# Sir-Teo/MuZero-Go

Measured on AMD Instinct MI355X. Metric: MCTS simulations/sec (whole node) + self-play moves/sec, 9x9 Go, 200 sims/move, higher is better.
Workload: dtype fp32

## Files before the change

include/mzgo.h:

```cpp
#ifndef MZGO_H
#define MZGO_H

#include <stdint.h>

#ifdef __cplusplus
extern "C" {
#endif

enum {
  MZGO_OK = 0,
  MZGO_EINVAL = -1,
  MZGO_EHIP = -2,
  MZGO_ENOWEIGHTS = -3,
  MZGO_EASSERT = -4
};

typedef struct mzgo_config {
  int board_size;
  int latent_dim;
  int num_games;
  int num_simulations;
  int max_moves;
  int compat;
  int temperature_moves;
// ... 45 lines not shown
int mzgo_board_reset(mzgo_engine* eng, void* stream);
int mzgo_board_step(mzgo_engine* eng, const int32_t* actions, int32_t* status, double* winner,
                    void* stream);
int mzgo_board_planes(mzgo_engine* eng, double* planes, void* stream);
int mzgo_board_set(mzgo_engine* eng, int g, const int8_t* stones_host, const uint8_t* invd_host,
                   const int32_t* meta_host, void* stream);

int mzgo_selfplay_reset(mzgo_engine* eng, int epoch, void* stream);
int mzgo_selfplay_move(mzgo_engine* eng, void* stream);
int mzgo_selfplay_moves(mzgo_engine* eng, int moves, void* stream);

int mzgo_arena_move(mzgo_engine* eng, mzgo_engine* opponent, void* stream);
int mzgo_arena_moves(mzgo_engine* eng, mzgo_engine* opponent, int moves, void* stream);
int mzgo_selfplay_counters(mzgo_engine* eng, uint64_t* counters_host, void* stream);
int mzgo_search_stats(mzgo_engine* eng, uint64_t* stats_host, void* stream);

int mzgo_selfplay_set_timing(mzgo_engine* eng, int on);
int mzgo_selfplay_launch_times(mzgo_engine* eng, float* boards_ms, float* queue_ms, int cap, int* n_host);
int mzgo_stream_wait_started(mzgo_engine* eng, uint64_t target, void* stream);
int mzgo_tower_timing(mzgo_engine* eng, int enable, double* tower_ms_host, int64_t* towers_host);

int mzgo_dyn_conv_backward_workspace(int B, int C, int64_t* bytes_host);
int mzgo_dyn_conv_backward(const float* grad_out, const float* out, const float* latent, const int64_t* action,
                           const float* emb, const float* weight, int B, int C, int N, float* grad_latent,
                           float* grad_weight, float* grad_bias, void* workspace, int64_t workspace_bytes,
                           void* stream);
int mzgo_conv3x3_relu_forward(const float* x, const int64_t* action, const float* emb, const float* weight,
                              const float* bias, int B, int Cin, int Cout, int N, float* out, void* stream);
int mzgo_conv3x3_backward_workspace(int B, int Cin, int Cout, int64_t* bytes_host);
int mzgo_conv3x3_backward(const float* grad_out, const float* out, const float* x, const int64_t* action,
// ... 67 lines not shown
```

muzero-go_amd/csrc/mzgo_capi.hip:

```cpp
#include <hip/hip_runtime.h>

#include <algorithm>
#include <cmath>
#include <cstdarg>
#include <cstdio>
#include <cstring>
#include <map>
#include <string>
#include <vector>

#include "../../include/mzgo.h"
#include "mzgo_dispatch.hpp"
#include "mzgo_replay.hpp"
#include "mzgo_tower_host.hpp"

namespace mzgo {
extern const KernelSet kernels_n5_c96, kernels_n6_c96, kernels_n9_c96, kernels_n19_c96, kernels_n6_c128,
    kernels_n6_c64;

size_t conv_bwd_workspace_bytes(int B, int Cin, int Cout);
hipError_t conv_forward(const float* x, const int64_t* action, const float* emb, const float* w, const float* bias,
                        int B, int Cin, int Cout, int N, float* y, hipStream_t s);
hipError_t conv_backward(const float* g, const float* out, const float* x, const int64_t* action, const float* emb,
                         const float* w, int B, int Cin, int Cout, int N, float* gx, float* gw, float* gb,
// ... 169 lines not shown
  float* d_w = nullptr;
  size_t d_w_bytes = 0;
  NetParams np{};
  EngineArrays E{};
  int* d_err = nullptr;
  unsigned* rq_head = nullptr;
  float* d_scr = nullptr;
  size_t scr_floats = 0;
  std::vector<void*> allocs;
  bool timing = false;
  std::vector<hipEvent_t> tev;
  int tn = 0;
  int64_t bytes = 0;
  int epoch = 0;
  int value_cache = 0;
  const double* noise = nullptr;
  double* noise_out = nullptr;
  TowerHost* tower = nullptr;

  template <class T>
  int alloc(T** p, size_t n) {
    void* v = nullptr;
    hipError_t e = hipMalloc(&v, n * sizeof(T) + 256);
    if (e != hipSuccess) return fail(MZGO_EHIP, "hipMalloc(%zu): %s", n * sizeof(T), hipGetErrorString(e));
    allocs.push_back(v);
    bytes += (int64_t)(n * sizeof(T));
    *p = reinterpret_cast<T*>(v);
    return MZGO_OK;
  }
  ~mzgo_engine() {
// ... 96 lines not shown

  SearchParams search_params() const {
    SearchParams sp;
    sp.c_puct = cfg.c_puct; sp.discount = cfg.discount;
    sp.dirichlet_alpha = cfg.dirichlet_alpha; sp.dirichlet_epsilon = cfg.dirichlet_epsilon;
    sp.pass_epsilon = cfg.pass_epsilon; sp.num_simulations = S; sp.compat = cfg.compat;
    sp.variant = cfg.search_variant;
    sp.factored = cfg.direct_dynamics ? 0 : 1;
    sp.seed = cfg.seed;
    sp.helpers = 0;
    sp.net = 0;
    sp.tail = 0;
    const char* lz = getenv("MZGO_LAZY_ROWS");
    sp.lazy_rows = lz && atoi(lz) == 0 ? 0 : 1;
    sp.value_cache = value_cache;
    return sp;
  }
};

void mzgo::replay_engine_view(const mzgo_engine* e, ReplayEngineView* v) {
  const EngineArrays& E = e->E;
  *v = ReplayEngineView{e->N, e->G, e->M, e->C, e->tower ? 1 : 0, e->cfg.game_base, e->epoch,
                        E.stones, E.invd, E.meta, E.rec_stones, E.rec_invd, E.rec_flags, E.rec_action,
                        E.rec_value, E.rec_policy, E.rec_reward, E.final_reward};
}

extern "C" {

const char* mzgo_last_error(void) { return g_err.c_str(); }

// ... 119 lines not shown
    }
  }
  if (C != 0) {
    chk(e->alloc(&E.prior, TSL * n1 * A));
    chk(e->alloc(&E.child, TSL * n1 * A));
    chk(e->alloc(&E.visits, TSL * n1));
    chk(e->alloc(&E.wsum, TSL * n1));
    chk(e->alloc(&E.root_prior, TSL * A));
    chk(e->alloc(&E.path, TSL * (n1 + 1)));
    chk(e->alloc(&E.nodes, TSL));
    chk(e->alloc(&E.nact, TSL * n1));
    const char* vc = getenv("MZGO_VALUE_CACHE");
    e->value_cache = !TW && !cfg->direct_dynamics && ks->value_cache_cap > 0 && e->S + 2 <= ks->value_cache_cap &&
                     !(vc && atoi(vc) == 0);
    if (e->value_cache) chk(e->alloc(&E.cval, TSL * n1 * A));
    chk(e->alloc(&E.jobs, TSL * job_bytes(A)));
    chk(e->alloc(&E.mpq, 2 * (size_t)G + 1));
    chk(e->alloc(&E.rec_stones, G * M * CELLS));
    chk(e->alloc(&E.rec_invd, G * M * CELLS));
    chk(e->alloc(&E.rec_flags, G * M));
    chk(e->alloc(&E.rec_action, G * M));
    chk(e->alloc(&E.rec_value, G * M));
    chk(e->alloc(&E.rec_policy, G * M * A));
    chk(e->alloc(&E.rec_reward, G * M));
  }
  chk(e->alloc(&E.stones, G * CELLS));
  chk(e->alloc(&E.invd, G * CELLS));
  chk(e->alloc(&E.meta, G * 4));
  chk(e->alloc(&E.game_len, G));
  chk(e->alloc(&E.final_reward, G));
// ... 499 lines not shown
    return fail(MZGO_EHIP, "mzgo_stream_wait_started: %llu gate(s) gave up before the target count", c[8]);
  }
  return MZGO_OK;
}

int mzgo_search_stats(mzgo_engine* e, uint64_t* out, void* stream) {
  if (!e || !out) return fail(MZGO_EINVAL, "bad argument");
  hipStream_t s = (hipStream_t)stream;
  unsigned long long c[3] = {};
  HIPCHK(hipMemcpyAsync(c, e->E.counters + 9, sizeof c, hipMemcpyDeviceToHost, s));
  HIPCHK(hipStreamSynchronize(s));
  out[0] = c[0]; out[1] = c[1]; out[2] = c[2];
  return MZGO_OK;
}

int mzgo_records_export(mzgo_engine* e, int g, int32_t* length, int32_t* status, int8_t* stones,
                        uint8_t* invd, uint8_t* flags, int32_t* action, double* value, double* policy,
                        double* reward, double* final_reward, void* stream) {
  if (!e || e->C == 0 || g < 0 || g >= e->G) return fail(MZGO_EINVAL, "bad argument");
  hipStream_t s = (hipStream_t)stream;
  int meta[4], st = 0;
  HIPCHK(hipMemcpyAsync(meta, e->E.meta + (size_t)g * 4, 16, hipMemcpyDeviceToHost, s));
  HIPCHK(hipMemcpyAsync(&st, e->E.status + g, 4, hipMemcpyDeviceToHost, s));
  HIPCHK(hipStreamSynchronize(s));
  if (int rc = check_chain(e, s)) return rc;
  const int L = meta[3];
  if (length) *length = L;
  if (status) *status = st;
  const size_t M = e->M, CELLS = e->CELLS, A = e->A, base = (size_t)g * M;
  if (L > 0) {
// ... 64 lines not shown
```

muzero-go_amd/csrc/mzgo_kernels.hpp:

```cpp
#pragma once
#include "mzgo_jobs.hpp"
#include "mzgo_replay.hpp"

namespace mzgo {

template <class G>
constexpr bool rep_needs_scratch() {
  if constexpr (G::WINO) return Wino<G>::NSTRIP > 1;
  else return false;
}

struct NoRepJobs {
  __device__ bool operator()(int) const { return false; }
};

template <class G, class PlaneFn, class Jobs = NoRepJobs>
__device__ __forceinline__ void representation(Smem<G>& sm, const NetParams& np, PlaneFn planes, float* lat,
                                      int lat_stride, float* scr, unsigned long long* ts = nullptr,
                                      Jobs jobs = Jobs{}) {
  float* mid = rep_needs_scratch<G>() ? scr : lat;
  for (int i = tid_local(); i < 6 * G::CELLS; i += G::THREADS) {
    const int c = i / G::CELLS, j = i - c * G::CELLS;
    sm.u.in[c * G::CPAD + j] = planes(c, j);
  }
// ... 814 lines not shown
  int* nact = E.nact + (size_t)g * ((size_t)E.S + 1);
  const int S = sp.num_simulations;
  const bool factored = sp.factored != 0;
  constexpr bool BATCH = decltype(sm.u.f)::BATCH;
  Acc T(TV, sm.t);
  tree_reset_root<G>(T);
  if (tid_local() == 0) {
    sm.t.newest = -1; sm.t.newp_node = -1; sm.t.ycache = -1; sm.t.rowc_node = -1; sm.t.lognode = -1;
  }
  __syncthreads();

  int nodes = 1, convs = 0;
  constexpr bool VCACHE = Acc::LDS && BATCH && decltype(sm.u.f)::CACHE;
  const bool vcache = VCACHE && factored && sp.value_cache != 0 && E.cval != nullptr && !shared_jobs<G>(sp);
  int nbcomp = 0, nbcache = 0, ncut = 0;
  auto cache_cut = [&](int leaf, int m, int B) {
    double* cv = E.cval + ((size_t)g * ((size_t)E.S + 1) + (size_t)leaf) * G::A;
    for (int i = m + tid_local() - 64; tid_local() >= 64 && i < B; i += G::THREADS - 64)
      cv[sm.u.f.acts[i]] = sm.u.f.bv[i];
    if (tid_local() == 0) sm.t.cvm[leaf >> 5] |= 1u << (leaf & 31);
    __syncthreads();
  };
  int rows = 0;
  const bool eager_rows = !(Acc::LDS || shared_jobs<G>(sp) || (decltype(sm.u.f)::GLOBAL_Y && sp.lazy_rows));
  Stamp st(E.stamps);
  int sim = 0;
  if (factored) {
    sim = root_batch<G, Acc>(sm, np, sp, E, g, TV, T, pool, scratch, nact, key, &st);
    if (eager_rows) rows += sim;
    nodes += sim;
// ... 3 lines not shown
  bool pending = false;
  int node0 = 0, depth0 = 0;
  while (sim < S) {
    if (!pending) {
      if (wave_id() == 0) {
        const int a = select_leaf<G>(sm.t, T, sp, key, sim, &st, node0, depth0);
        if (lane_id_local() == 0) sm.t.action = a;
        st.wave_add(92, 1);
        st.wave_add(95, (unsigned long long)sm.t.depth);
      }
      __syncthreads();
    }
    pending = false;
    node0 = 0;
    depth0 = 0;
    while (sm.t.action == kNeedLogits) {
      const int xn = sm.t.leaf, xd = sm.t.depth;
      st.lap(0);
      if (y_lds_target<G>(sm) != nullptr && sm.t.ycache == sm.t.lpar)
        policy_sums_wg<G>(sm.t.logits, sm.u.f.yc, np.etab + (size_t)sm.t.lact * 9 * G::C, sm.u.f.hw);
      else
        policy_sums_wg<G>(sm.t.logits, pool + (size_t)sm.t.lpar * node_floats,
                          np.etab + (size_t)sm.t.lact * 9 * G::C, np.head_w);
      if (tid_local() == 0) sm.t.lognode = xn;
      ++rows;
      __syncthreads();
      st.lap(32);
      if (tid_local() == 0) st.wave_add(34, 1);
      if (wave_id() == 0) {
        const int a = select_leaf<G>(sm.t, T, sp, key, sim, &st, xn, xd);
        if (lane_id_local() == 0) sm.t.action = a;
      }
      __syncthreads();
      st.lap(33);
    }
    st.lap(0);
    const int a = sm.t.action, leaf = sm.t.leaf, depth = sm.t.depth;
    if (a < 0) {
      if (wave_id() == 0 && a == -1) backup<G>(T, depth, -1, 0.0);
      __syncthreads();
      ++sim;
      continue;
    }
    const float* heads;
    const int nid = nodes;
    if (factored) {
      float* yleaf = pool + (size_t)leaf * node_floats;
      int yc = sm.t.ycache;
      bool prepicked = false;
      static_assert(!decltype(sm.u.f)::CACHE || 3 * G::C <= G::THREADS, "one head weight per thread");
      float hwpre = 0.f;
      bool hwready = false;
      if (!sm.t.yready) {
        const bool sj = shared_jobs<G>(sp);
        if (leaf != 0 && !sj && !G::WINO) {
          const int par = T.path(depth - 1);
          materialize<G>(scratch, pool + (size_t)par * node_floats, np.etab + (size_t)nact[leaf] * 9 * G::C,
                         sm.ulds());
        }
        st.lap(81);
        if (sj) {
          const int nun0 = sm.t.nunexp, B0 = BATCH ? (nun0 < S - sim ? nun0 : S - sim) : 1;
          prepicked = BATCH && B0 >= 2;
          conv_shared<G>(sm, np, E, g, leaf, sp.net, &st, leaf != 0 ? T.path(depth - 1) : -1,
                         leaf != 0 ? nact[leaf] : 0, [&](unsigned cb) {
                           if (prepicked && wave_id() == 0) {
                             uint64_t um0[G::AP];
#pragma unroll
// ... 6 lines not shown
        } else if (G::WINO && leaf != 0) {
          const int par = T.path(depth - 1);
          if constexpr (decltype(sm.u.f)::CACHE) hwpre = tid_local() < 3 * G::C ? np.head_w[tid_local()] : 0.f;
          bool tail = false;
          if constexpr (TailConvs<G>::value) {
            if (sp.tail) {
              if (tid_local() == 0)
                sm.bc[3] = __hip_atomic_load(&job_of<G>(E, g).h->nhelp, __ATOMIC_RELAXED, __HIP_MEMORY_SCOPE_AGENT) > 0;
              __syncthreads();
              tail = sm.bc[3] != 0;
            }
          }
          if (tail) {
            conv_tail<G>(sm, np, E, g, leaf, par, nact[leaf], sp.net, y_lds_target<G>(sm),
                         y_lds_target<G>(sm) != nullptr && yc == par, &st);
          } else {
            latent_conv_rebuilt<G>(sm, np, pool + (size_t)par * node_floats, np.etab + (size_t)nact[leaf] * 9 * G::C,
                                   yleaf, &st, y_lds_target<G>(sm), y_lds_target<G>(sm) != nullptr && yc == par);
          }
          hwready = true;
        } else {
          latent_conv<G, G::C, G::C, 0, true>(sm, np.w_dyn, np.b_dyn, scratch, G::CS, nullptr, yleaf, G::CS,
                                              G::CS, nullptr, &st, G::WINO ? y_lds_target<G>(sm) : nullptr);
        }
        __syncthreads();
        st.lap(82);
        if (!sj && G::WINO && y_lds_target<G>(sm) != nullptr) {
          if (hwready) {
            if (tid_local() < 3 * G::C) sm.u.f.hw[tid_local()] = hwpre;
          } else {
            load_hw<G>(sm, np.head_w);
          }
          if (tid_local() == 0) sm.t.ycache = leaf;
          yc = leaf;
          const int nun1 = sm.t.nunexp;
          if (!(BATCH && (nun1 < S - sim ? nun1 : S - sim) >= 2)) __syncthreads();
        } else {
          yc = -1;
        }
        if (tid_local() == 0) { st.wave_add(59, 1); ++convs; }
      }
// ... 159 lines not shown
      backup<G>(T, depth, nid, (double)r + sp.discount * (double)v, sp.variant == 0);
    }
    st.lap(3);
    ++sim;
  }
  __syncthreads();
  st.flush();
  tree_flush<G>(T, nodes);
  if (tid_local() == 0) {
    E.nodes[g] = nodes;
    atomicAdd(&E.counters[3], (unsigned long long)(factored ? convs : nodes - 1));
    atomicAdd(&E.counters[5], (unsigned long long)(factored ? rows : nodes - 1));
    if (nbcomp) atomicAdd(&E.counters[9], (unsigned long long)nbcomp);
    if (nbcache) atomicAdd(&E.counters[10], (unsigned long long)nbcache);
    if (ncut) atomicAdd(&E.counters[11], (unsigned long long)ncut);
  }
  __syncthreads();
}

template <class G, class PlaneFn>
__device__ __forceinline__ void run_search(Smem<G>& sm, const NetParams& np, const SearchParams& sp,
                                  const EngineArrays& E, int g, PlaneFn planes, const double* noise,
                                  uint64_t key, unsigned long long* ts = nullptr, double* noise_out = nullptr) {
  const TreeView TV = TreeViewOf<G>::make(E, g);
  if (tid_local() == 0) sm.t.ngrab = 0;
  build_mask<G>(sm.t, sp.pass_epsilon, [&](int a) { return planes(3, a); });
  float* pool = pool_of<G>(E, g);
  const size_t node_floats = (size_t)G::C * G::CS;
  if (sp.factored && shared_jobs<G>(sp))
    representation<G>(sm, np, planes, pool + (size_t)(E.S + 1) * node_floats, G::CS, pool, ts ? ts + 3 : nullptr,
// ... 490 lines not shown
```

muzero-go_amd/csrc/mzgo_move.hpp:

```cpp
#pragma once
#include "mzgo_board.hpp"
#include "mzgo_search.hpp"

namespace mzgo {

constexpr int kCounters = 12;

struct EngineArrays {
  int S;
  int max_moves;
  float* pool;
  float* prior;
  int* child;
  int* visits;
  double* wsum;
  double* root_prior;
  int* path;
  int* nodes;
  int* nact;
  double* cval;
  int8_t* stones;
  uint8_t* invd;
  int* meta;
  int8_t* rec_stones;
// ... 293 lines not shown
```

muzero-go_amd/csrc/mzgo_search.hpp:

```cpp
#pragma once
#include "mzgo_common.hpp"
#include <type_traits>

namespace mzgo {

struct SearchParams {
  double c_puct;
  double discount;
  double dirichlet_alpha;
  double dirichlet_epsilon;
  double pass_epsilon;
  int num_simulations;
  int compat;
  int variant;
  int factored;
  uint64_t seed;
  int helpers;
  int net;
  int tail;
  int lazy_rows;
  int value_cache;
};

struct TreeView {
  float* prior;
  int* child;
  int* visits;
  double* wsum;
  double* root_prior;
  int* path;
};

constexpr int kRawRow = -2;
constexpr int kLazyRow = -3;
constexpr int kNeedLogits = -4;

// ... 616 lines not shown
  if (!(best_s > -INFINITY)) return -1;
  int best_a = -1;
#pragma unroll
  for (int j = 0; j < G::AP; ++j) {
    const uint64_t hit = __ballot(sc[j] == best_s);
    if (best_a < 0 && hit) {
      const int l = __ffsll((long long)hit) - 1;
      best_a = 64 * j + l;
      best_c = __builtin_amdgcn_readlane(ch[j], l);
    }
  }
  return best_a;
}

template <class G, class Acc>
__device__ __forceinline__ int select_leaf(TreeLds<G>& t, const Acc& T, const SearchParams& sp,
                                  uint64_t key, int sim, Stamp* st = nullptr, int node0 = 0, int depth0 = 0) {
  const int lane = lane_id_local();
  int node = node0, depth = depth0, par = -1, pact = -1;
  if (st) { st->lap(35); st->wave_add(51, 1); }
#ifdef MZGO_STAMPS
  asm volatile("s_waitcnt vmcnt(0)" ::: "memory");
  if (st) st->lap(38);
#endif
  auto need_logits = [&]() {
    t.leaf = node; t.depth = depth; t.lpar = par; t.lact = pact;
    return kNeedLogits;
  };
  for (int guard = 0; guard <= sp.num_simulations + 1; ++guard) {
    const bool root = node == 0;
// ... 25 lines not shown
#pragma unroll
      for (int j = 0; j < G::AP; ++j) {
        const int a = lane + 64 * j;
        P[j] = a < G::A ? (double)t.newp[a] : 0.0;
        ch[j] = -1;
      }
    } else if (Acc::LDS && node == t.rowc_node) {
#pragma unroll
      for (int j = 0; j < G::AP; ++j) {
        const int a = lane + 64 * j;
        P[j] = a < G::A ? (double)t.rowc_prior[a] : 0.0;
        ch[j] = a < G::A ? t.rowc_child[a] : -1;
      }
    } else if (t.is_raw(node)) {
      if (t.lognode != node) return need_logits();
      if (t.newest >= 0)
        while (__hip_atomic_load(&t.newp_node, __ATOMIC_ACQUIRE, __HIP_MEMORY_SCOPE_WORKGROUP) != t.newest)
          __builtin_amdgcn_s_sleep(1);
      float q[G::AP];
      if (st) st->lap(36);
      settle_lazy<G>(t, const_cast<float*>(pr_row), T.T.child + (size_t)node * G::A, sp.variant, t.fbuf, t.dbuf, q);
      if (lane == 0) atomicAnd(&t.rawp[node >> 5], ~(1u << (node & 31)));
      if (st) { st->lap(49); st->wave_add(50, 1); }
#pragma unroll
      for (int j = 0; j < G::AP; ++j) {
        const int a = lane + 64 * j;
        P[j] = a < G::A ? (double)q[j] : 0.0;
        ch[j] = -1;
        if constexpr (Acc::LDS)
          if (a < G::A) { t.rowc_prior[a] = q[j]; t.rowc_child[a] = -1; }
      }
      if constexpr (Acc::LDS)
        if (lane == 0) t.rowc_node = node;
    } else {
      hbm_rows = true;
#pragma unroll
      for (int j = 0; j < G::AP; ++j) {
        const int a = lane + 64 * j;
        P[j] = a < G::A ? (double)pr_row[a] : 0.0;
        ch[j] = a < G::A ? T.T.child[(size_t)node * G::A + a] : -1;
      }
      if constexpr (!Acc::LDS) {
        const int c0 = __builtin_amdgcn_readfirstlane(ch[0]);
        if (c0 == kLazyRow) {
          if (t.lognode != node) return need_logits();
          if (t.newest >= 0)
            while (__hip_atomic_load(&t.newp_node, __ATOMIC_ACQUIRE, __HIP_MEMORY_SCOPE_WORKGROUP) != t.newest)
              __builtin_amdgcn_s_sleep(1);
// ... 148 lines not shown
```

muzero-go_amd/csrc/mzgo_smem.hpp:

```cpp
#pragma once
#include "mzgo_board.hpp"
#include "mzgo_conv.hpp"
#include "mzgo_expand.hpp"
#include "mzgo_move.hpp"
#include "mzgo_search.hpp"
#include "mzgo_wino.hpp"

namespace mzgo {

struct NetParams {
  const float* w_conv1; const float* b_conv1;
  const float* w_conv2; const float* b_conv2;
  const float* w_conv3; const float* b_conv3;
  const float* w_dyn;   const float* b_dyn;
  const float* emb;
  const float* head_w;
  const float* etab;
  HeadScalars hs;
};

__device__ __forceinline__ NetParams select_params(bool b, const NetParams& x, const NetParams& y) {
  NetParams n;
#define MZGO_SEL(f) n.f = b ? x.f : y.f;
  MZGO_SEL(w_conv1) MZGO_SEL(b_conv1) MZGO_SEL(w_conv2) MZGO_SEL(b_conv2) MZGO_SEL(w_conv3) MZGO_SEL(b_conv3)
// ... 140 lines not shown
    for (int s = 0; s < Wino<G>::NSTRIP; ++s) {
      wino_input<G, CIN>(sm.u.v, sm.raw, src, src_stride, emb, s, st);
      if (st) st->lap(1);
      wino_conv<G, CIN, COUT, NH, YM>(sm.u.v, sm.u.x.red, sm.u.x.hp, sm.u.x.outs, sm.hfin, w, b, dst, dst_stride,
                                  out_cells, head_w, s, st, ylds);
    }
    if constexpr (Wino<G>::NSTRIP > 1) __syncthreads();
  } else {
    stage_board<G>(sm.u.in, src, src_stride, CIN, emb);
    __syncthreads();
    if (st) st->lap(1);
    conv3x3_ring<G, CIN, COUT, NH, YM>(sm.u.in, sm.ring, w, b, dst, dst_stride, out_cells, head_w, sm.u.hp, st);
  }
}

template <class G>
__device__ __forceinline__ void latent_conv_rebuilt(Smem<G>& sm, const NetParams& np, const float* ypar,
                                                    const float* ea, float* dst, Stamp* st = nullptr,
                                                    float* ylds = nullptr, bool par_in_lds = false) {
  if constexpr (G::WINO && Wino<G>::NSTRIP == 1) {
    wino_conv_rebuilt<G>(sm.u.v, sm.raw, sm.u.x.red, sm.u.x.hp, sm.u.x.outs, sm.hfin, ypar, ea, np.w_dyn, np.b_dyn,
                         dst, st, ylds, par_in_lds ? ylds : nullptr);
  } else if constexpr (G::WINO) {
    for (int s = 0; s < Wino<G>::NSTRIP; ++s)
      wino_conv_rebuilt<G>(sm.u.v, sm.raw, sm.u.x.red, sm.u.x.hp, sm.u.x.outs, sm.hfin, ypar, ea, np.w_dyn,
                           np.b_dyn, dst, st, ylds, par_in_lds ? ylds : nullptr, s);
    if constexpr (Wino<G>::NSTRIP > 1) __syncthreads();
  }
}

template <class G>
__device__ __forceinline__ BoardLds<G> board_lds(Smem<G>& sm) {
  return make_board_lds<G>(sm.stone, sm.invd, sm.u.scr.label, sm.u.scr.libs, sm.u.scr.gsize, sm.killed, sm.misc);
}

template <class G>
__device__ __forceinline__ float* pool_of(const EngineArrays& E, int g) {
// ... 20 lines not shown
```

muzero-go_amd/csrc/mzgo_wino.hpp:

```cpp
#pragma once
#include "mzgo_common.hpp"


namespace mzgo {
constexpr int kWinoXG = 2;
}

namespace mzgo {

template <class G>
struct Wino {
  static constexpr int TY = (G::N + 1) / 2;
  static constexpr int TX = (G::N + 2) / 3;
  static constexpr int TRS = (16 / TX < TY) ? 16 / TX : TY;
  static constexpr int NSTRIP = (TY + TRS - 1) / TRS;
  static constexpr int T = TRS * TX;
  static constexpr int SROWS = 2 * TRS;
  static constexpr int SCELLS = SROWS * G::N;
  static constexpr int XI = 20;
  static_assert(T <= 16, "a strip's tiles must fit one MFMA column tile");
  static constexpr int LAST_C0 = (NSTRIP - 1) * SCELLS;
  static constexpr int OCELLS = SCELLS > G::CS - LAST_C0 ? SCELLS : G::CS - LAST_C0;
  static constexpr int OUT_STRIDE = OCELLS + (36 - OCELLS % 32) % 32;
  static_assert(OUT_STRIDE > OCELLS, "junk cell past the stored row");
// ... 274 lines not shown
}

__device__ __forceinline__ constexpr float wino_at2(int oy, int i) {
  return oy == 0 ? (i < 3 ? 1.f : 0.f) : (i == 0 ? 0.f : (i == 2 ? -1.f : 1.f));
}
__device__ __forceinline__ constexpr float wino_at3(int ox, int j) {
  return ox == 0 ? (j < 4 ? 1.f : 0.f)
                 : (ox == 1 ? (j == 0 ? 0.f : (j == 1 ? 1.f : (j == 2 ? -1.f : (j == 3 ? -2.f : 0.f))))
                            : (j == 0 ? 0.f : (j == 3 ? 4.f : 1.f)));
}

struct WinoNoHook {
  static constexpr bool DEFERS = false;
  __device__ void operator()(int) const {}
  __device__ void finish() const {}
};
template <class G, int CIN, int COUT, int NH, bool YM = false, class Hook = WinoNoHook>
__device__ __forceinline__ void wino_conv(const float* V, float* red, float* hp, float* outs, float* hfin,
                                          const float* __restrict__ upk,
                                          const float* __restrict__ bias, float* __restrict__ out,
                                          int out_stride, int out_cells, const float* __restrict__ head_w,
                                          int strip = 0, Stamp* st = nullptr, float* ylds = nullptr, int m0 = 0,
                                          int nm = COUT / 16, Hook hook = Hook{}) {
  typedef Wino<G> W;
  constexpr int CH = CIN / 2, S4 = CH / 16, MT = COUT / 16, XI = W::XI;
  constexpr int OS = W::OUT_STRIDE;
  constexpr int XH = XI / 2;
  constexpr int KP = CIN / 16;
  constexpr int L = XH * KP;
  constexpr int PF = 8;
// ... 60 lines not shown
          } else if (kh == 0 && !Hook::DEFERS) {
#pragma unroll
            for (int q = 0; q < XG; ++q) bn[q] = bp[bidx(q, KH)];
          }
          __builtin_amdgcn_sched_barrier(0);
#pragma unroll
          for (int e = 0; e < 4; ++e)
#pragma unroll
            for (int q = 0; q < XG; ++q)
              acc[g * XG + q] = __builtin_amdgcn_mfma_f32_16x16x4f32(a[q][e], b[q][e], acc[g * XG + q], 0, 0, 0);
#pragma unroll
          for (int q = 0; q < XG; ++q)
            if (pos0 + q + PF < L) ar[(pos0 + q) % PF] = ap[(pos0 + q + PF) * 64];
          __builtin_amdgcn_sched_barrier(0);
          if (kh == 0) hook(s);
        }
      }
    }
#pragma unroll
    for (int xl = 0; xl < XH; ++xl) {
      const int il = xl / 5, j = xl % 5;
      const f32x4 mv = acc[xl];
#pragma unroll
      for (int ox = 0; ox < 3; ++ox) {
        const float cf = wino_at3(ox, j);
        if (cf == 1.f) yp[il * 3 + ox] += mv;
        else if (cf == -1.f) yp[il * 3 + ox] -= mv;
        else if (cf != 0.f) yp[il * 3 + ox] += cf * mv;
      }
    }
// ... 196 lines not shown
        const int co = i / Q, q = i - co * Q;
        const f32x4 v = *reinterpret_cast<const f32x4*>(outs + co * OS + q * 4);
        f32x4* dst = reinterpret_cast<f32x4*>(out + (size_t)co * G::CS + c0) + q;
        __builtin_nontemporal_store(v, dst);
      }
    } else {
      const int n = min(c0 + W::SCELLS, out_cells) - c0;
      for (int i = tid_local(); i < COUT * n; i += G::THREADS) {
        const int co = i / n, j = i - co * n;
        out[(size_t)co * out_stride + c0 + j] = outs[co * OS + j];
      }
    }
  }
}

template <class G>
struct RebuiltHook {
  static constexpr bool DEFERS = true;
  static constexpr int kScatter = 2, kBarrier = 7, kTransform = 10;
  RebuiltInput<G, G::C> in;
  __device__ __forceinline__ void operator()(int s) {
    if (s == kScatter) in.scatter(1);
    else if (s == kBarrier) __syncthreads();
    else if (s == kTransform) in.transform(1);
  }
  __device__ __forceinline__ void finish() { __syncthreads(); }
};
template <class G>
__device__ __forceinline__ void wino_conv_rebuilt(float* V, float* raw, float* red, float* hp, float* outs,
                                                  float* hfin, const float* __restrict__ ypar,
                                                  const float* __restrict__ ea, const float* __restrict__ upk,
                                                  const float* __restrict__ bias, float* __restrict__ out,
                                                  Stamp* st, float* ylds, const float* ysrc_lds, int strip = 0,
                                                  int m0 = 0, int nm = G::C / 16) {
  static_assert(RebuiltInput<G, G::C>::SLABS == 2, "two slabs");
  RebuiltInput<G, G::C> in(V, raw, ypar, ea, strip, ysrc_lds);
  in.begin();
  in.slab(0);
  if (st) st->lap(1);
  wino_conv<G, G::C, G::C, 0, true, RebuiltHook<G>>(V, red, hp, outs, hfin, upk, bias, out, G::CS, G::CS, nullptr,
                                                     strip, st, ylds, m0, nm, RebuiltHook<G>{in});
}

}
```

muzero-go_amd/mzgo/_lib.py:

```python
import ctypes
import os

import torch

LIB_PATH = os.environ.get("MZGO_LIB") or os.path.join(os.path.dirname(os.path.abspath(__file__)), "libmzgo.so")

MZGO_OK, MZGO_EINVAL, MZGO_EHIP, MZGO_ENOWEIGHTS, MZGO_EASSERT = 0, -1, -2, -3, -4


class Config(ctypes.Structure):

    _fields_ = [
        ("board_size", ctypes.c_int),
        ("latent_dim", ctypes.c_int),
        ("num_games", ctypes.c_int),
        ("num_simulations", ctypes.c_int),
        ("max_moves", ctypes.c_int),
        ("compat", ctypes.c_int),
        ("temperature_moves", ctypes.c_int),
        ("search_variant", ctypes.c_int),
        ("c_puct", ctypes.c_double),
        ("discount", ctypes.c_double),
        ("dirichlet_alpha", ctypes.c_double),
        ("dirichlet_epsilon", ctypes.c_double),
# ... 24 lines not shown
    "mzgo_check_inference_errors": (_I, [_P, _P]),
    "mzgo_search": (_I, [_P, _P, _P, _I, _I, _P, _P, _P]),
    "mzgo_reanalyse": (_I, [_P, _P, _P, _P, _P, _P, _I, _P, _P, _P, _P]),
    "mzgo_tree_export": (_I, [_P, _I, _P, _P, _P, _P, _P, _P, _P]),
    "mzgo_board_reset": (_I, [_P, _P]),
    "mzgo_board_step": (_I, [_P, _P, _P, _P, _P]),
    "mzgo_board_planes": (_I, [_P, _P, _P]),
    "mzgo_board_set": (_I, [_P, _I, _P, _P, _P, _P]),
    "mzgo_selfplay_reset": (_I, [_P, _I, _P]),
    "mzgo_selfplay_move": (_I, [_P, _P]),
    "mzgo_selfplay_moves": (_I, [_P, _I, _P]),
    "mzgo_arena_move": (_I, [_P, _P, _P]),
    "mzgo_arena_moves": (_I, [_P, _P, _I, _P]),
    "mzgo_selfplay_counters": (_I, [_P, _P, _P]),
    "mzgo_search_stats": (_I, [_P, _P, _P]),
    "mzgo_selfplay_set_timing": (_I, [_P, _I]),
    "mzgo_selfplay_launch_times": (_I, [_P, _P, _P, _I, _P]),
    "mzgo_stream_wait_started": (_I, [_P, ctypes.c_uint64, _P]),
    "mzgo_tower_timing": (_I, [_P, _I, _P, _P]),
    "mzgo_selfplay_inject_noise": (_I, [_P, _P]),
    "mzgo_selfplay_record_noise": (_I, [_P, _P]),
    "mzgo_tower_record_nodes": (_I, [_P, _P]),
    "mzgo_records_export": (_I, [_P, _I, _P, _P, _P, _P, _P, _P, _P, _P, _P, _P, _P]),
    "mzgo_records_pack": (_I, [_P, _P, ctypes.c_int64, _P, _P]),
    "mzgo_dyn_conv_backward_workspace": (_I, [_I, _I, ctypes.POINTER(ctypes.c_int64)]),
    "mzgo_dyn_conv_backward": (_I, [_P, _P, _P, _P, _P, _P, _I, _I, _I, _P, _P, _P, _P, ctypes.c_int64, _P]),
    "mzgo_conv3x3_relu_forward": (_I, [_P, _P, _P, _P, _P, _I, _I, _I, _I, _P, _P]),
    "mzgo_conv3x3_backward_workspace": (_I, [_I, _I, _I, ctypes.POINTER(ctypes.c_int64)]),
    "mzgo_conv3x3_backward": (_I, [_P, _P, _P, _P, _P, _P, _I, _I, _I, _I, _P, _P, _P, _P, ctypes.c_int64, _P]),
    "mzgo_replay_create": (_I, [_I, _I, _I, _I, ctypes.POINTER(_P)]),
# ... 70 lines not shown
```

muzero-go_amd/mzgo/engine.py:

```python
import ctypes
from dataclasses import dataclass, fields

import numpy as np
import torch

from . import _lib
from ._lib import check, lib, ptr, stream_of


@dataclass
class EngineConfig:

    board_size: int = 9
    latent_dim: int = 96
    num_games: int = 1
    num_simulations: int = 128
    max_moves: int = 0
    compat: str = "reference"
    temperature_moves: int = 15
    search_variant: str = "self_play"
    c_puct: float = 2.5
    discount: float = 0.99
    dirichlet_alpha: float = 0.15
    dirichlet_epsilon: float = 0.02
# ... 209 lines not shown
        q = np.zeros(cap, np.float32)
        n = ctypes.c_int()
        check(lib.mzgo_selfplay_launch_times(self._h, ptr(b), ptr(q), cap, ctypes.byref(n)))
        check(lib.mzgo_selfplay_set_timing(self._h, int(enable)))
        k = min(n.value, cap)
        return b[:k].tolist(), q[:k].tolist()

    def counters(self):
        out = np.zeros(9, np.uint64)
        check(lib.mzgo_selfplay_counters(self._h, ptr(out), stream_of(self.device)))
        return dict(simulations=int(out[0]), moves=int(out[1]), games_finished=int(out[2]),
                    playing=int(out[3]), dynamics_convs=int(out[4]), tail_convs=int(out[5]),
                    prior_rows=int(out[6]), workgroups_started=int(out[7]), tail_wait_expiries=int(out[8]))

    def search_stats(self):
        out = np.zeros(3, np.uint64)
        check(lib.mzgo_search_stats(self._h, ptr(out), stream_of(self.device)))
        return dict(batch_children_computed=int(out[0]), batch_children_cached=int(out[1]), batches_cut=int(out[2]))

    def wait_started(self, target, stream=None):
        s = stream if stream is not None else torch.cuda.current_stream(self.device)
        check(lib.mzgo_stream_wait_started(self._h, int(target), ctypes.c_void_p(s.cuda_stream)))

    def record(self, g):
        M, CELLS, A = self.M, self.N * self.N, self.A
        length = ctypes.c_int32()
        status = ctypes.c_int32()
        stones = np.empty((M, CELLS), np.int8)
        invd = np.empty((M, CELLS), np.uint8)
        flags = np.empty(M, np.uint8)
        action = np.empty(M, np.int32)
        value = np.empty(M, np.float64)
        policy = np.empty((M, A), np.float64)
# ... 10 lines not shown
```

Measured before the change: 137.9 million.

## Overlap leaf policy logits and arrival selection with the dynamics convolution

When search reaches a raw leaf that needs logits, it no longer runs a separate logits pass followed by a later dynamics conv. It now enters the Winograd rebuilt conv directly and computes the policy sums in a pre-hook. The lazy-prior settle and child selection run in a mid-conv hook on wave 0, so logits, settle and the conv overlap inside one pass instead of running serially. New counters for these arrival convs are exposed through a new stats API. The risk is extra register and LDS pressure in the conv, plus hook-ordering hazards around the shared tree state.

```diff
diff --git a/include/mzgo.h b/include/mzgo.h
--- a/include/mzgo.h
+++ b/include/mzgo.h
@@ -83,6 +83,7 @@
 int mzgo_arena_moves(mzgo_engine* eng, mzgo_engine* opponent, int moves, void* stream);
 int mzgo_selfplay_counters(mzgo_engine* eng, uint64_t* counters_host, void* stream);
 int mzgo_search_stats(mzgo_engine* eng, uint64_t* stats_host, void* stream);
+int mzgo_search_stats2(mzgo_engine* eng, uint64_t* stats_host, int cap, void* stream);
 
 int mzgo_selfplay_set_timing(mzgo_engine* eng, int on);
 int mzgo_selfplay_launch_times(mzgo_engine* eng, float* boards_ms, float* queue_ms, int cap, int* n_host);
diff --git a/muzero-go_amd/csrc/mzgo_capi.hip b/muzero-go_amd/csrc/mzgo_capi.hip
--- a/muzero-go_amd/csrc/mzgo_capi.hip
+++ b/muzero-go_amd/csrc/mzgo_capi.hip
@@ -207,6 +207,7 @@
   int64_t bytes = 0;
   int epoch = 0;
   int value_cache = 0;
+  int arrival_conv = 1;
   const double* noise = nullptr;
   double* noise_out = nullptr;
   TowerHost* tower = nullptr;
@@ -333,6 +334,7 @@
     const char* lz = getenv("MZGO_LAZY_ROWS");
     sp.lazy_rows = lz && atoi(lz) == 0 ? 0 : 1;
     sp.value_cache = value_cache;
+    sp.arrival_conv = arrival_conv;
     return sp;
   }
 };
@@ -482,6 +484,8 @@
     e->value_cache = !TW && !cfg->direct_dynamics && ks->value_cache_cap > 0 && e->S + 2 <= ks->value_cache_cap &&
                      !(vc && atoi(vc) == 0);
     if (e->value_cache) chk(e->alloc(&E.cval, TSL * n1 * A));
+    const char* ac = getenv("MZGO_ARRIVAL_CONV");
+    e->arrival_conv = !(ac && atoi(ac) <= 0);
     chk(e->alloc(&E.jobs, TSL * job_bytes(A)));
     chk(e->alloc(&E.mpq, 2 * (size_t)G + 1));
     chk(e->alloc(&E.rec_stones, G * M * CELLS));
@@ -1011,6 +1015,17 @@
   return MZGO_OK;
 }
 
+int mzgo_search_stats2(mzgo_engine* e, uint64_t* out, int cap, void* stream) {
+  if (!e || !out || cap < 0) return fail(MZGO_EINVAL, "bad argument");
+  hipStream_t s = (hipStream_t)stream;
+  constexpr int n = kCounters - 9;
+  unsigned long long c[n] = {};
+  HIPCHK(hipMemcpyAsync(c, e->E.counters + 9, sizeof c, hipMemcpyDeviceToHost, s));
+  HIPCHK(hipStreamSynchronize(s));
+  for (int i = 0; i < (cap < n ? cap : n); ++i) out[i] = c[i];
+  return MZGO_OK;
+}
+
 int mzgo_records_export(mzgo_engine* e, int g, int32_t* length, int32_t* status, int8_t* stones,
                         uint8_t* invd, uint8_t* flags, int32_t* action, double* value, double* policy,
                         double* reward, double* final_reward, void* stream) {
diff --git a/muzero-go_amd/csrc/mzgo_kernels.hpp b/muzero-go_amd/csrc/mzgo_kernels.hpp
--- a/muzero-go_amd/csrc/mzgo_kernels.hpp
+++ b/muzero-go_amd/csrc/mzgo_kernels.hpp
@@ -852,6 +852,10 @@
   constexpr bool VCACHE = Acc::LDS && BATCH && decltype(sm.u.f)::CACHE;
   const bool vcache = VCACHE && factored && sp.value_cache != 0 && E.cval != nullptr && !shared_jobs<G>(sp);
   int nbcomp = 0, nbcache = 0, ncut = 0;
+  constexpr bool ARRIVAL = Acc::LDS && BATCH && G::WINO && decltype(sm.u.f)::CACHE && Wino<G>::NSTRIP == 1;
+  const bool arrival = ARRIVAL && factored && sp.arrival_conv != 0 && sp.variant == 0 && !sp.tail &&
+                       !shared_jobs<G>(sp);
+  int narr_lds = 0, narr_l2 = 0;
   auto cache_cut = [&](int leaf, int m, int B) {
     double* cv = E.cval + ((size_t)g * ((size_t)E.S + 1) + (size_t)leaf) * G::A;
     for (int i = m + tid_local() - 64; tid_local() >= 64 && i < B; i += G::THREADS - 64)
@@ -885,7 +889,9 @@
     pending = false;
     node0 = 0;
     depth0 = 0;
+    bool arrive = false;
     while (sm.t.action == kNeedLogits) {
+      if (arrival) { arrive = true; break; }
       const int xn = sm.t.leaf, xd = sm.t.depth;
       st.lap(0);
       if (y_lds_target<G>(sm) != nullptr && sm.t.ycache == sm.t.lpar)
@@ -906,8 +912,9 @@
       st.lap(33);
     }
     st.lap(0);
-    const int a = sm.t.action, leaf = sm.t.leaf, depth = sm.t.depth;
-    if (a < 0) {
+    int a = sm.t.action;
+    const int leaf = sm.t.leaf, depth = sm.t.depth;
+    if (a < 0 && !arrive) {
       if (wave_id() == 0 && a == -1) backup<G>(T, depth, -1, 0.0);
       __syncthreads();
       ++sim;
@@ -922,7 +929,7 @@
       static_assert(!decltype(sm.u.f)::CACHE || 3 * G::C <= G::THREADS, "one head weight per thread");
       float hwpre = 0.f;
       bool hwready = false;
-      if (!sm.t.yready) {
+      if (arrive || !sm.t.yready) {
         const bool sj = shared_jobs<G>(sp);
         if (leaf != 0 && !sj && !G::WINO) {
           const int par = T.path(depth - 1);
@@ -959,6 +966,31 @@
           if (tail) {
             conv_tail<G>(sm, np, E, g, leaf, par, nact[leaf], sp.net, y_lds_target<G>(sm),
                          y_lds_target<G>(sm) != nullptr && yc == par, &st);
+          } else if constexpr (ARRIVAL) {
+            const float* ypar = pool + (size_t)par * node_floats;
+            const float* ea = np.etab + (size_t)nact[leaf] * 9 * G::C;
+            latent_conv_rebuilt<G>(
+                sm, np, ypar, ea, yleaf, &st, y_lds_target<G>(sm), yc == par,
+                [&]() {
+                  if (arrive) {
+                    if (yc == par) policy_sums_wg<G>(sm.t.logits, sm.u.f.yc, ea, sm.u.f.hw);
+                    else policy_sums_wg<G>(sm.t.logits, ypar, ea, np.head_w);
+                  }
+                },
+                [&]() {
+                  if (arrive && __builtin_amdgcn_readfirstlane(wave_id()) == 0) {
+                    const unsigned long long t_a = st.now();
+                    if (lane_id_local() == 0) sm.t.lognode = leaf;
+                    const int ax = settle_arrival<G>(sm.t, T, sp, key, sim, nullptr, leaf, depth);
+                    if (lane_id_local() == 0) sm.t.action = ax;
+                    st.wave_add(49, st.now() - t_a);
+                    st.wave_add(50, 1);
+                  }
+                });
+            if (arrive) {
+              ++rows;
+              if (yc == par) ++narr_lds; else ++narr_l2;
+            }
           } else {
             latent_conv_rebuilt<G>(sm, np, pool + (size_t)par * node_floats, np.etab + (size_t)nact[leaf] * 9 * G::C,
                                    yleaf, &st, y_lds_target<G>(sm), y_lds_target<G>(sm) != nullptr && yc == par);
@@ -970,6 +1002,7 @@
         }
         __syncthreads();
         st.lap(82);
+        if (arrive) a = sm.t.action;
         if (!sj && G::WINO && y_lds_target<G>(sm) != nullptr) {
           if (hwready) {
             if (tid_local() < 3 * G::C) sm.u.f.hw[tid_local()] = hwpre;
@@ -1159,6 +1192,8 @@
     if (nbcomp) atomicAdd(&E.counters[9], (unsigned long long)nbcomp);
     if (nbcache) atomicAdd(&E.counters[10], (unsigned long long)nbcache);
     if (ncut) atomicAdd(&E.counters[11], (unsigned long long)ncut);
+    if (narr_lds) atomicAdd(&E.counters[12], (unsigned long long)narr_lds);
+    if (narr_l2) atomicAdd(&E.counters[13], (unsigned long long)narr_l2);
   }
   __syncthreads();
 }
diff --git a/muzero-go_amd/csrc/mzgo_move.hpp b/muzero-go_amd/csrc/mzgo_move.hpp
--- a/muzero-go_amd/csrc/mzgo_move.hpp
+++ b/muzero-go_amd/csrc/mzgo_move.hpp
@@ -4,7 +4,7 @@
 
 namespace mzgo {
 
-constexpr int kCounters = 12;
+constexpr int kCounters = 14;
 
 struct EngineArrays {
   int S;
diff --git a/muzero-go_amd/csrc/mzgo_search.hpp b/muzero-go_amd/csrc/mzgo_search.hpp
--- a/muzero-go_amd/csrc/mzgo_search.hpp
+++ b/muzero-go_amd/csrc/mzgo_search.hpp
@@ -20,6 +20,7 @@
   int tail;
   int lazy_rows;
   int value_cache;
+  int arrival_conv;
 };
 
 struct TreeView {
@@ -666,6 +667,59 @@
 }
 
 template <class G, class Acc>
+__device__ __forceinline__ int settle_arrival(TreeLds<G>& t, const Acc& T, const SearchParams& sp, uint64_t key,
+                                              int sim, Stamp* st, int node, int depth) {
+  const int lane = lane_id_local();
+  if (t.newest >= 0)
+    while (__hip_atomic_load(&t.newp_node, __ATOMIC_ACQUIRE, __HIP_MEMORY_SCOPE_WORKGROUP) != t.newest)
+      __builtin_amdgcn_s_sleep(1);
+  float q[G::AP];
+  if (st) st->lap(36);
+  settle_lazy<G>(t, T.T.prior + (size_t)node * G::A, T.T.child + (size_t)node * G::A, sp.variant, t.fbuf, t.dbuf, q);
+  if (lane == 0) atomicAnd(&t.rawp[node >> 5], ~(1u << (node & 31)));
+  if (st) { st->lap(49); st->wave_add(50, 1); }
+  double P[G::AP];
+#pragma unroll
+  for (int j = 0; j < G::AP; ++j) {
+    const int a = lane + 64 * j;
+    P[j] = a < G::A ? (double)q[j] : 0.0;
+    if constexpr (Acc::LDS)
+      if (a < G::A) { t.rowc_prior[a] = q[j]; t.rowc_child[a] = -1; }
+  }
+  if constexpr (Acc::LDS)
+    if (lane == 0) t.rowc_node = node;
+  uint64_t anypos = 0, unexp[G::AP];
+  int n_unexp = 0;
+#pragma unroll
+  for (int j = 0; j < G::AP; ++j) {
+    unexp[j] = __ballot(P[j] > 0.0);
+    anypos |= unexp[j];
+    n_unexp += __popcll(unexp[j]);
+  }
+  if (st) st->lap(36);
+  if (!anypos) { t.leaf = node; t.depth = depth; return sp.variant == 1 ? -2 : -1; }
+  uint32_t k = randbelow(draw(key, TAG_SELECT, (uint64_t)sim), (uint32_t)n_unexp);
+  int best = -1;
+#pragma unroll
+  for (int j = 0; j < G::AP; ++j) {
+    const uint32_t c = __popcll(unexp[j]);
+    if (best < 0 && k < c) {
+      best = 64 * j + kth_set_bit(unexp[j], k);
+    } else if (best < 0) {
+      k -= c;
+    }
+  }
+  t.leaf = node;
+  t.depth = depth;
+  t.yready = 0;
+  t.nunexp = n_unexp;
+#pragma unroll
+  for (int j = 0; j < G::AP; ++j) t.umask[j] = unexp[j];
+  if (st) st->lap(37);
+  return best;
+}
+
+template <class G, class Acc>
 __device__ __forceinline__ int select_leaf(TreeLds<G>& t, const Acc& T, const SearchParams& sp,
                                   uint64_t key, int sim, Stamp* st = nullptr, int node0 = 0, int depth0 = 0) {
   const int lane = lane_id_local();
@@ -721,24 +775,7 @@
       }
     } else if (t.is_raw(node)) {
       if (t.lognode != node) return need_logits();
-      if (t.newest >= 0)
-        while (__hip_atomic_load(&t.newp_node, __ATOMIC_ACQUIRE, __HIP_MEMORY_SCOPE_WORKGROUP) != t.newest)
-          __builtin_amdgcn_s_sleep(1);
-      float q[G::AP];
-      if (st) st->lap(36);
-      settle_lazy<G>(t, const_cast<float*>(pr_row), T.T.child + (size_t)node * G::A, sp.variant, t.fbuf, t.dbuf, q);
-      if (lane == 0) atomicAnd(&t.rawp[node >> 5], ~(1u << (node & 31)));
-      if (st) { st->lap(49); st->wave_add(50, 1); }
-#pragma unroll
-      for (int j = 0; j < G::AP; ++j) {
-        const int a = lane + 64 * j;
-        P[j] = a < G::A ? (double)q[j] : 0.0;
-        ch[j] = -1;
-        if constexpr (Acc::LDS)
-          if (a < G::A) { t.rowc_prior[a] = q[j]; t.rowc_child[a] = -1; }
-      }
-      if constexpr (Acc::LDS)
-        if (lane == 0) t.rowc_node = node;
+      return settle_arrival<G>(t, T, sp, key, sim, st, node, depth);
     } else {
       hbm_rows = true;
 #pragma unroll
diff --git a/muzero-go_amd/csrc/mzgo_smem.hpp b/muzero-go_amd/csrc/mzgo_smem.hpp
--- a/muzero-go_amd/csrc/mzgo_smem.hpp
+++ b/muzero-go_amd/csrc/mzgo_smem.hpp
@@ -178,13 +178,14 @@
   }
 }
 
-template <class G>
+template <class G, class Pre = WinoNoMid, class Mid = WinoNoMid>
 __device__ __forceinline__ void latent_conv_rebuilt(Smem<G>& sm, const NetParams& np, const float* ypar,
                                                     const float* ea, float* dst, Stamp* st = nullptr,
-                                                    float* ylds = nullptr, bool par_in_lds = false) {
+                                                    float* ylds = nullptr, bool par_in_lds = false,
+                                                    Pre pre = Pre{}, Mid mid = Mid{}) {
   if constexpr (G::WINO && Wino<G>::NSTRIP == 1) {
     wino_conv_rebuilt<G>(sm.u.v, sm.raw, sm.u.x.red, sm.u.x.hp, sm.u.x.outs, sm.hfin, ypar, ea, np.w_dyn, np.b_dyn,
-                         dst, st, ylds, par_in_lds ? ylds : nullptr);
+                         dst, st, ylds, par_in_lds ? ylds : nullptr, 0, 0, G::C / 16, pre, mid);
   } else if constexpr (G::WINO) {
     for (int s = 0; s < Wino<G>::NSTRIP; ++s)
       wino_conv_rebuilt<G>(sm.u.v, sm.raw, sm.u.x.red, sm.u.x.hp, sm.u.x.outs, sm.hfin, ypar, ea, np.w_dyn,
diff --git a/muzero-go_amd/csrc/mzgo_wino.hpp b/muzero-go_amd/csrc/mzgo_wino.hpp
--- a/muzero-go_amd/csrc/mzgo_wino.hpp
+++ b/muzero-go_amd/csrc/mzgo_wino.hpp
@@ -312,6 +312,7 @@
   static constexpr bool DEFERS = false;
   __device__ void operator()(int) const {}
   __device__ void finish() const {}
+  __device__ void second(int) const {}
 };
 template <class G, int CIN, int COUT, int NH, bool YM = false, class Hook = WinoNoHook>
 __device__ __forceinline__ void wino_conv(const float* V, float* red, float* hp, float* outs, float* hfin,
@@ -402,6 +403,7 @@
             if (pos0 + q + PF < L) ar[(pos0 + q) % PF] = ap[(pos0 + q + PF) * 64];
           __builtin_amdgcn_sched_barrier(0);
           if (kh == 0) hook(s);
+          else hook.second(g * KH + kk);
         }
       }
     }
@@ -628,32 +630,43 @@
   }
 }
 
-template <class G>
+struct WinoNoMid {
+  __device__ void operator()() const {}
+};
+template <class G, class Mid = WinoNoMid>
 struct RebuiltHook {
   static constexpr bool DEFERS = true;
   static constexpr int kScatter = 2, kBarrier = 7, kTransform = 10;
+  static constexpr int kArrive = 1;
   RebuiltInput<G, G::C> in;
+  Mid mid;
   __device__ __forceinline__ void operator()(int s) {
     if (s == kScatter) in.scatter(1);
     else if (s == kBarrier) __syncthreads();
     else if (s == kTransform) in.transform(1);
   }
   __device__ __forceinline__ void finish() { __syncthreads(); }
+  __device__ __forceinline__ void second(int s) {
+    if (s == kArrive) mid();
+  }
 };
-template <class G>
+template <class G, class Pre = WinoNoMid, class Mid = WinoNoMid>
 __device__ __forceinline__ void wino_conv_rebuilt(float* V, float* raw, float* red, float* hp, float* outs,
                                                   float* hfin, const float* __restrict__ ypar,
                                                   const float* __restrict__ ea, const float* __restrict__ upk,
                                                   const float* __restrict__ bias, float* __restrict__ out,
                                                   Stamp* st, float* ylds, const float* ysrc_lds, int strip = 0,
-                                                  int m0 = 0, int nm = G::C / 16) {
+                                                  int m0 = 0, int nm = G::C / 16, Pre pre = Pre{},
+                                                  Mid mid = Mid{}) {
   static_assert(RebuiltInput<G, G::C>::SLABS == 2, "two slabs");
   RebuiltInput<G, G::C> in(V, raw, ypar, ea, strip, ysrc_lds);
   in.begin();
+  pre();
   in.slab(0);
   if (st) st->lap(1);
-  wino_conv<G, G::C, G::C, 0, true, RebuiltHook<G>>(V, red, hp, outs, hfin, upk, bias, out, G::CS, G::CS, nullptr,
-                                                     strip, st, ylds, m0, nm, RebuiltHook<G>{in});
-}
-
-}
+  wino_conv<G, G::C, G::C, 0, true, RebuiltHook<G, Mid>>(V, red, hp, outs, hfin, upk, bias, out, G::CS, G::CS,
+                                                          nullptr, strip, st, ylds, m0, nm,
+                                                          RebuiltHook<G, Mid>{in, mid});
+}
+
+}
diff --git a/muzero-go_amd/mzgo/_lib.py b/muzero-go_amd/mzgo/_lib.py
--- a/muzero-go_amd/mzgo/_lib.py
+++ b/muzero-go_amd/mzgo/_lib.py
@@ -62,6 +62,7 @@
     "mzgo_arena_moves": (_I, [_P, _P, _I, _P]),
     "mzgo_selfplay_counters": (_I, [_P, _P, _P]),
     "mzgo_search_stats": (_I, [_P, _P, _P]),
+    "mzgo_search_stats2": (_I, [_P, _P, _I, _P]),
     "mzgo_selfplay_set_timing": (_I, [_P, _I]),
     "mzgo_selfplay_launch_times": (_I, [_P, _P, _P, _I, _P]),
     "mzgo_stream_wait_started": (_I, [_P, ctypes.c_uint64, _P]),
diff --git a/muzero-go_amd/mzgo/engine.py b/muzero-go_amd/mzgo/engine.py
--- a/muzero-go_amd/mzgo/engine.py
+++ b/muzero-go_amd/mzgo/engine.py
@@ -247,9 +247,10 @@
                     prior_rows=int(out[6]), workgroups_started=int(out[7]), tail_wait_expiries=int(out[8]))
 
     def search_stats(self):
-        out = np.zeros(3, np.uint64)
-        check(lib.mzgo_search_stats(self._h, ptr(out), stream_of(self.device)))
-        return dict(batch_children_computed=int(out[0]), batch_children_cached=int(out[1]), batches_cut=int(out[2]))
+        out = np.zeros(5, np.uint64)
+        check(lib.mzgo_search_stats2(self._h, ptr(out), len(out), stream_of(self.device)))
+        return dict(batch_children_computed=int(out[0]), batch_children_cached=int(out[1]), batches_cut=int(out[2]),
+                    arrival_convs_lds=int(out[3]), arrival_convs_l2=int(out[4]))
 
     def wait_started(self, target, stream=None):
         s = stream if stream is not None else torch.cuda.current_stream(self.device)
```

Measured after the change: 142.6 million (median of 6 runs). 1.03x the previous value.
